# MaxWolf-01/sentinel2-landcover-classification

Hardware: AMD Instinct MI355X
Metric: Sentinel-2 256x256x13 tiles/sec fwd+bwd (higher is better)
Workload: dtype f32

## Files before the change

### sentinel2-landcover-classification_amd/csrc/ew.hip

```cpp
#include "common.h"

namespace s2k {

constexpr int CHUNK = 4096;

template <typename T>
static T* ref_ptr(const Ctx& c, int64_t ref) {
    if (ref < 0) return nullptr;
    const int base = (int)(ref >> 56);
    const int64_t off = ref & ((1ll << 56) - 1);
    if (base >= c.n_bases || c.bases[base] == nullptr) return reinterpret_cast<T*>(1);
    return reinterpret_cast<T*>(static_cast<char*>(c.bases[base]) + off);
}
static bool bad(const void* q) { return q == reinterpret_cast<const void*>(1); }
#define CHECK_PTRS(name, ...)                                                                         \
    do {                                                                                              \
        const void* _ps[] = {__VA_ARGS__};                                                            \
        for (const void* _q : _ps)                                                                    \
            if (bad(_q)) { set_error(name ": tensor references a null base"); return S2K_EFAULT; }    \
    } while (0)

struct Task {
    int64_t plane;
    int start, count;
// ... 998 lines not shown
    if (!dgate || !gate || !hpre || !pool || !w1 || !w2 || !dpool || !hs || B <= 0 || (params && (!dw1 || !db1 || !dw2 || !db2))) {
        set_error("se_fc_bwd: bad args"); return S2K_EINVAL;
    }
    if (Q > 8192 || B > 65535) { set_error("se_fc_bwd: C/Q too large"); return S2K_EINVAL; }
    if ((size_t)(C + 1024) * 4 > 64000) { set_error("se_fc_bwd: C too large"); return S2K_EINVAL; }
    if (Q <= 64) {
        hipLaunchKernelGGL(se_fc_bwd_small_kernel, dim3(B), dim3(1024), (size_t)(C + 1024 + 64) * sizeof(float), c.stream, dgate, gate, hpre, w1, w2,
                           hs, dpool, C, Q);
    } else {
    hipLaunchKernelGGL(se_fc_bwd_a1_kernel, dim3(cdiv(Q, 64), B), dim3(1024), (C + 1024) * sizeof(float), c.stream, dgate, gate, hpre, w2, hs, B, C, Q);
    hipLaunchKernelGGL(se_fc_bwd_a2_kernel, dim3(cdiv(C, NTHREADS), B), dim3(NTHREADS), Q * sizeof(float), c.stream, dgate, gate, hpre, w1, dpool, B, C, Q);
    }
    if (!params) return S2K_OK;
    launch_se_fc_param_grads(dgate, hs, hpre, pool, dw1, db1, dw2, db2, B, C, Q, c.stream);
    return S2K_OK;
}

int launch_se_fc_wgrad(const S2kOp& op, const Ctx& c) {
    const float* dgp = ref_ptr<const float>(c, op.t[S2K_SE_FC_WGRAD_T_DGP]);
    const float* hs = ref_ptr<const float>(c, op.t[S2K_SE_FC_WGRAD_T_HS]);
    const float* dhp = ref_ptr<const float>(c, op.t[S2K_SE_FC_WGRAD_T_DHP]);
    const float* pool = ref_ptr<const float>(c, op.t[S2K_SE_FC_WGRAD_T_POOL]);
    float* dw1 = ref_ptr<float>(c, op.t[S2K_SE_FC_WGRAD_T_DW1]);
    float* db1 = ref_ptr<float>(c, op.t[S2K_SE_FC_WGRAD_T_DB1]);
    float* dw2 = ref_ptr<float>(c, op.t[S2K_SE_FC_WGRAD_T_DW2]);
    float* db2 = ref_ptr<float>(c, op.t[S2K_SE_FC_WGRAD_T_DB2]);
    CHECK_PTRS("se_fc_wgrad", dgp, hs, dhp, pool, dw1, db1, dw2, db2);
    const int B = op.d[S2K_SE_FC_WGRAD_D_B], C = op.d[S2K_SE_FC_WGRAD_D_C], Q = op.d[S2K_SE_FC_WGRAD_D_CSQ];
    if (!dgp || !hs || !dhp || !pool || !dw1 || !db1 || !dw2 || !db2 || B <= 0 || C <= 0 || Q <= 0) { set_error("se_fc_wgrad: bad args"); return S2K_EINVAL; }
    launch_se_fc_param_grads(dgp, hs, dhp, pool, dw1, db1, dw2, db2, B, C, Q, c.stream);
    return S2K_OK;
}

template <bool VEC>
__global__ void __launch_bounds__(NTHREADS) bn_bwd_reduce_kernel(const float* g, const float* y, const float* bnv,
                                                                 const float* mulbc, const float* addbc, const float* noise,
                                                                 float* gout, double* stats2, int C, int HW, int64_t nplanes,
                                                                 int act, float keep, float addscale, int nrep) {
    Task t;
    if (!get_task(HW, nplanes, t)) return;
    const int lane = threadIdx.x & 63;
    const int c = (int)((uint32_t)t.plane % (uint32_t)C);
    const int b = (int)((uint32_t)t.plane / (uint32_t)C);
    const float scale = bnv[c], shift = bnv[C + c], mean = bnv[2 * C + c], invstd = bnv[3 * C + c];
    float mul = mulbc ? mulbc[t.plane] : 1.0f;
    if (noise) mul *= floorf(keep + noise[b]) / keep;
    const float add = addbc ? addbc[t.plane] * addscale : 0.0f;
    const int64_t base = t.plane * HW + t.start;
    float s1 = 0.0f, s2 = 0.0f;
    if (VEC) {
        const int n4 = t.count >> 2;
        for (int i = lane; i < n4; i += 64) {
            float4 gv = reinterpret_cast<const float4*>(g + base)[i];
            const float4 yv = reinterpret_cast<const float4*>(y + base)[i];
            float* gp = &gv.x;
            const float* yp = &yv.x;
#pragma unroll
            for (int k = 0; k < 4; ++k) {
                float v = fmaf(gp[k], mul, add);
                if (act != S2K_PRO_NONE) v *= act_grad(fmaf(yp[k], scale, shift), act);
                gp[k] = v;
                s1 += v;
                s2 = fmaf(v, (yp[k] - mean) * invstd, s2);
            }
            reinterpret_cast<float4*>(gout + base)[i] = gv;
        }
    } else {
        for (int i = lane; i < t.count; i += 64) {
            const float yy = y[base + i];
            float v = fmaf(g[base + i], mul, add);
            if (act != S2K_PRO_NONE) v *= act_grad(fmaf(yy, scale, shift), act);
            gout[base + i] = v;
            s1 += v;
            s2 = fmaf(v, (yy - mean) * invstd, s2);
        }
    }
    s1 = wave_sum(s1);
    s2 = wave_sum(s2);
    if (lane == 0) {
        double* st = stats2 + (int64_t)(blockIdx.x % nrep) * 2 * C;
        atomic_add_d(st + c, (double)s1);
        atomic_add_d(st + C + c, (double)s2);
    }
}

int launch_bn_bwd_reduce(const S2kOp& op, const Ctx& c) {
    const float* g = ref_ptr<const float>(c, op.t[S2K_BN_BWD_REDUCE_T_G]);
    const float* y = ref_ptr<const float>(c, op.t[S2K_BN_BWD_REDUCE_T_Y]);
    const float* bnv = ref_ptr<const float>(c, op.t[S2K_BN_BWD_REDUCE_T_BNV]);
    const float* mulbc = ref_ptr<const float>(c, op.t[S2K_BN_BWD_REDUCE_T_MULBC]);
    const float* addbc = ref_ptr<const float>(c, op.t[S2K_BN_BWD_REDUCE_T_ADDBC]);
    const float* noise = ref_ptr<const float>(c, op.t[S2K_BN_BWD_REDUCE_T_NOISE]);
    float* gout = ref_ptr<float>(c, op.t[S2K_BN_BWD_REDUCE_T_GOUT]);
    double* st2 = ref_ptr<double>(c, op.t[S2K_BN_BWD_REDUCE_T_STATS2]);
    CHECK_PTRS("bn_bwd_reduce", g, y, bnv, mulbc, addbc, noise, gout, st2);
    const int B = op.d[S2K_BN_BWD_REDUCE_D_B], C = op.d[S2K_BN_BWD_REDUCE_D_C], HW = op.d[S2K_BN_BWD_REDUCE_D_HW];
    if (!g || !y || !bnv || !gout || !st2 || B <= 0 || C <= 0 || HW <= 0) { set_error("bn_bwd_reduce: bad args"); return S2K_EINVAL; }
    const int64_t nplanes = (int64_t)B * C;
    const unsigned blocks = task_blocks(HW, nplanes);
    const int act = op.d[S2K_BN_BWD_REDUCE_D_ACT];
    const float keep = op.f[S2K_BN_BWD_REDUCE_F_KEEP], addscale = op.f[S2K_BN_BWD_REDUCE_F_ADDSCALE];
    const int nrep = op.d[S2K_BN_BWD_REDUCE_D_NREP] > 0 ? op.d[S2K_BN_BWD_REDUCE_D_NREP] : 1;
    if ((HW & 3) == 0)
        hipLaunchKernelGGL((bn_bwd_reduce_kernel<true>), dim3(blocks), dim3(NTHREADS), 0, c.stream, g, y, bnv, mulbc, addbc, noise,
                           gout, st2, C, HW, nplanes, act, keep, addscale, nrep);
    else
        hipLaunchKernelGGL((bn_bwd_reduce_kernel<false>), dim3(blocks), dim3(NTHREADS), 0, c.stream, g, y, bnv, mulbc, addbc, noise,
                           gout, st2, C, HW, nplanes, act, keep, addscale, nrep);
    return S2K_OK;
}

__global__ void bn_bwd_finalize_kernel(const double* st2, const float* gamma, const float* bnv, float* dgamma, float* dbeta,
                                       float* coef, int C, double count, int nrep) {
    const int c = blockIdx.x * 4 + (threadIdx.x >> 6);
    const int lane = threadIdx.x & 63;
    if (c >= C) return;
    double s1 = 0.0, s2 = 0.0;
    for (int r = lane; r < nrep; r += 64) { s1 += st2[(int64_t)r * 2 * C + c]; s2 += st2[(int64_t)r * 2 * C + C + c]; }
    s1 = wave_sum_d(s1);
    s2 = wave_sum_d(s2);
    if (lane != 0) return;
    dgamma[c] += (float)s2;
    dbeta[c] += (float)s1;
    const double a = (double)gamma[c] * (double)bnv[3 * C + c];
    coef[c] = (float)a;
    coef[C + c] = (float)(-a * s2 / count);
    coef[2 * C + c] = (float)(-a * s1 / count);
}

int launch_bn_bwd_finalize(const S2kOp& op, const Ctx& c) {
    const double* st2 = ref_ptr<const double>(c, op.t[S2K_BN_BWD_FINALIZE_T_STATS2]);
    const float* gamma = ref_ptr<const float>(c, op.t[S2K_BN_BWD_FINALIZE_T_GAMMA]);
    const float* bnv = ref_ptr<const float>(c, op.t[S2K_BN_BWD_FINALIZE_T_BNV]);
    float* dgamma = ref_ptr<float>(c, op.t[S2K_BN_BWD_FINALIZE_T_DGAMMA]);
    float* dbeta = ref_ptr<float>(c, op.t[S2K_BN_BWD_FINALIZE_T_DBETA]);
    float* coef = ref_ptr<float>(c, op.t[S2K_BN_BWD_FINALIZE_T_COEF]);
    CHECK_PTRS("bn_bwd_finalize", st2, gamma, bnv, dgamma, dbeta, coef);
    const int C = op.d[S2K_BN_BWD_FINALIZE_D_C];
    if (!st2 || !gamma || !bnv || !dgamma || !dbeta || !coef || C <= 0) { set_error("bn_bwd_finalize: bad args"); return S2K_EINVAL; }
    hipLaunchKernelGGL(bn_bwd_finalize_kernel, dim3(cdiv(C, 4)), dim3(256), 0, c.stream, st2, gamma, bnv, dgamma, dbeta, coef, C,
                       (double)op.n[S2K_BN_BWD_FINALIZE_N_COUNT], op.d[S2K_BN_BWD_FINALIZE_D_NREP] > 0 ? op.d[S2K_BN_BWD_FINALIZE_D_NREP] : 1);
    return S2K_OK;
}

struct BnFuse {
    const double* st2;
    const float* gamma;
    float *dgamma, *dbeta;
    double inv_count;
    int nrep;
    const float *mulbc, *addbc;
    float addscale;
    const float* ps;
    int B;
};

__device__ __forceinline__ void bn_fuse_sums(const BnFuse& fz, int C, int c, int lane, double& s1, double& s2) {
    s1 = 0.0; s2 = 0.0;
    if (fz.ps) {
        const int64_t np = (int64_t)fz.B * C;
        for (int b = lane; b < fz.B; b += 64) {
            const int64_t pl = (int64_t)b * C + c;
            const double mul = fz.mulbc ? (double)fz.mulbc[pl] : 1.0, add = fz.addbc ? (double)fz.addbc[pl] * (double)fz.addscale : 0.0;
            s1 += mul * (double)fz.ps[pl] + add * (double)fz.ps[np + pl];
            s2 += mul * (double)fz.ps[2 * np + pl] + add * (double)fz.ps[3 * np + pl];
        }
        s1 = wave_sum_d(s1);
        s2 = wave_sum_d(s2);
    } else if (fz.nrep <= 8) {
        for (int r = 0; r < fz.nrep; ++r) { s1 += fz.st2[(int64_t)r * 2 * C + c]; s2 += fz.st2[(int64_t)r * 2 * C + C + c]; }
    } else {
        for (int r = lane; r < fz.nrep; r += 64) { s1 += fz.st2[(int64_t)r * 2 * C + c]; s2 += fz.st2[(int64_t)r * 2 * C + C + c]; }
        s1 = wave_sum_d(s1);
        s2 = wave_sum_d(s2);
    }
}

__device__ __forceinline__ uint32_t pm_pk_bf16(float lo, float hi) {
    typedef __bf16 b2 __attribute__((ext_vector_type(2)));
    typedef float f2 __attribute__((ext_vector_type(2)));
    f2 v = {lo, hi};
    return __builtin_bit_cast(uint32_t, __builtin_convertvector(v, b2));
}

template <int MODE, bool VEC, bool OUT16 = false>
__global__ void __launch_bounds__(NTHREADS) plane_map_kernel(const float* a, const float* y, const float* bnv, const float* coef,
                                                             const float* noise, float* out, int C, int HW, int64_t nplanes,
                                                             float keep, const BnFuse fz, const BnFold fold = BnFold{}) {
    Task t;
    if (!get_task(HW, nplanes, t)) return;
    const int lane = threadIdx.x & 63;
    const int c = (int)((uint32_t)t.plane % (uint32_t)C);
    const int64_t base = t.plane * HW + t.start;
    float4 av0 = make_float4(0, 0, 0, 0), yv0 = make_float4(0, 0, 0, 0);
    if (VEC && lane < (t.count >> 2)) {
        if (a) av0 = reinterpret_cast<const float4*>(a + base)[lane];
        yv0 = reinterpret_cast<const float4*>(y + base)[lane];
    }
    float k0, k1, k2;
    float gmul = 1.0f, gadd = 0.0f, bscale = 1.0f, bshift = 0.0f;
    if (MODE == 3) {
        gmul = fz.mulbc ? fz.mulbc[t.plane] : 1.0f;
        gadd = fz.addbc ? fz.addbc[t.plane] * fz.addscale : 0.0f;
        bscale = bnv[c];
        bshift = bnv[C + c];
    }
    if (MODE >= 2) {
        double s1, s2;
        bn_fuse_sums(fz, C, c, lane, s1, s2);
        const float mean = bnv[2 * C + c], invstd = bnv[3 * C + c];
        const double aa = (double)fz.gamma[c] * (double)invstd;
        const float A = (float)aa, Bq = (float)(-aa * s2 * fz.inv_count), Cq = (float)(-aa * s1 * fz.inv_count);
        k0 = A; k1 = Bq * invstd; k2 = Cq - Bq * invstd * mean;
        if (t.plane < C && t.start == 0 && lane == 0) {
            fz.dgamma[c] += (float)s2;
            fz.dbeta[c] += (float)s1;
        }
    } else if (MODE == 0) {
        const float mean = bnv[2 * C + c], invstd = bnv[3 * C + c];
        const float A = coef[c], Bq = coef[C + c], Cq = coef[2 * C + c];
        k0 = A; k1 = Bq * invstd; k2 = Cq - Bq * invstd * mean;
    } else {
        float dcs = 1.0f;
        if (noise) dcs = floorf(keep + noise[(int)(t.plane / C)]) / keep;
        float sc, sh;
        if (fold.stats) bn_fold_wave(fold, C, c, t.plane < C && t.start == 0, sc, sh);
        else { sc = bnv[c]; sh = bnv[C + c]; }
        k0 = a ? 1.0f : 0.0f; k1 = sc * dcs; k2 = sh * dcs;
    }
    if (VEC) {
        const int n4 = t.count >> 2;
        for (int i = lane; i < n4; i += 64) {
            float4 av = av0, yv = yv0;
            if (i + 64 < n4) {
                if (a) av0 = reinterpret_cast<const float4*>(a + base)[i + 64];
                yv0 = reinterpret_cast<const float4*>(y + base)[i + 64];
            }
            if (MODE == 3) {
                av.x = fmaf(av.x, gmul, gadd) * act_grad(fmaf(yv.x, bscale, bshift), S2K_PRO_SILU);
                av.y = fmaf(av.y, gmul, gadd) * act_grad(fmaf(yv.y, bscale, bshift), S2K_PRO_SILU);
                av.z = fmaf(av.z, gmul, gadd) * act_grad(fmaf(yv.z, bscale, bshift), S2K_PRO_SILU);
                av.w = fmaf(av.w, gmul, gadd) * act_grad(fmaf(yv.w, bscale, bshift), S2K_PRO_SILU);
            }
            float4 o;
            o.x = fmaf(k0, av.x, fmaf(k1, yv.x, k2)); o.y = fmaf(k0, av.y, fmaf(k1, yv.y, k2));
            o.z = fmaf(k0, av.z, fmaf(k1, yv.z, k2)); o.w = fmaf(k0, av.w, fmaf(k1, yv.w, k2));
            if constexpr (OUT16) reinterpret_cast<uint2*>(reinterpret_cast<uint16_t*>(out) + base)[i] = make_uint2(pm_pk_bf16(o.x, o.y), pm_pk_bf16(o.z, o.w));
            else reinterpret_cast<float4*>(out + base)[i] = o;
        }
    } else {
        for (int i = lane; i < t.count; i += 64) {
            float av = a ? a[base + i] : 0.0f;
            if (MODE == 3) av = fmaf(av, gmul, gadd) * act_grad(fmaf(y[base + i], bscale, bshift), S2K_PRO_SILU);
            out[base + i] = fmaf(k0, av, fmaf(k1, y[base + i], k2));
        }
    }
}

template <int MODE, bool OUT16 = false>
__global__ void __launch_bounds__(NTHREADS) bn_bwd_apply_small_kernel(const float* a, const float* y, const float* bnv, float* out,
                                                                      int B, int C, int HW, int lpp, const BnFuse fz) {
    const int lane = threadIdx.x & 63;
    const int c = blockIdx.x * 4 + (threadIdx.x >> 6);
    if (c >= C) return;
    double s1, s2;
    bn_fuse_sums(fz, C, c, lane, s1, s2);
    const float mean = bnv[2 * C + c], invstd = bnv[3 * C + c];
    const double aa = (double)fz.gamma[c] * (double)invstd;
    const float A = (float)aa, Bq = (float)(-aa * s2 * fz.inv_count), Cq = (float)(-aa * s1 * fz.inv_count);
    const float k0 = A, k1 = Bq * invstd, k2 = Cq - Bq * invstd * mean;
    if (blockIdx.y == 0 && lane == 0) {
        fz.dgamma[c] += (float)s2;
        fz.dbeta[c] += (float)s1;
    }
    const float bscale = bnv[c], bshift = bnv[C + c];
    const int pp = 64 / lpp, sub = lane / lpp, li = lane & (lpp - 1);
    if (4 * li >= HW) return;
    const int bper = (B + gridDim.y - 1) / gridDim.y, b_lo = blockIdx.y * bper, b_hi = min(B, b_lo + bper);
    constexpr int U = 4;
    for (int b0 = b_lo + sub; b0 < b_hi; b0 += pp * U) {
        float4 av[U], yv[U];
        float gmul[U], gadd[U];
#pragma unroll
        for (int u = 0; u < U; ++u) {
            const int b = min(b0 + u * pp, b_hi - 1);
            const int64_t plane = (int64_t)b * C + c, off = plane * HW + 4 * li;
            av[u] = *reinterpret_cast<const float4*>(a + off);
            yv[u] = *reinterpret_cast<const float4*>(y + off);
            gmul[u] = 1.0f;
            gadd[u] = 0.0f;
            if (MODE == 3) {
                if (fz.mulbc) gmul[u] = fz.mulbc[plane];
                if (fz.addbc) gadd[u] = fz.addbc[plane] * fz.addscale;
            }
        }
#pragma unroll
        for (int u = 0; u < U; ++u) {
            const int b = b0 + u * pp;
            if (b >= b_hi) break;
            float4 g = av[u];
            const float4 yy = yv[u];
            if (MODE == 3) {
                g.x = fmaf(g.x, gmul[u], gadd[u]) * act_grad(fmaf(yy.x, bscale, bshift), S2K_PRO_SILU);
                g.y = fmaf(g.y, gmul[u], gadd[u]) * act_grad(fmaf(yy.y, bscale, bshift), S2K_PRO_SILU);
                g.z = fmaf(g.z, gmul[u], gadd[u]) * act_grad(fmaf(yy.z, bscale, bshift), S2K_PRO_SILU);
                g.w = fmaf(g.w, gmul[u], gadd[u]) * act_grad(fmaf(yy.w, bscale, bshift), S2K_PRO_SILU);
            }
            float4 o;
            o.x = fmaf(k0, g.x, fmaf(k1, yy.x, k2)); o.y = fmaf(k0, g.y, fmaf(k1, yy.y, k2));
            o.z = fmaf(k0, g.z, fmaf(k1, yy.z, k2)); o.w = fmaf(k0, g.w, fmaf(k1, yy.w, k2));
            if constexpr (OUT16) *reinterpret_cast<uint2*>(reinterpret_cast<uint16_t*>(out) + ((int64_t)b * C + c) * HW + 4 * li) = make_uint2(pm_pk_bf16(o.x, o.y), pm_pk_bf16(o.z, o.w));
            else *reinterpret_cast<float4*>(out + ((int64_t)b * C + c) * HW + 4 * li) = o;
        }
    }
}

template <int MODE, bool OUT16 = false>
static bool launch_bn_bwd_apply_small(const float* a, const float* y, const float* bnv, float* out, int B, int C, int HW,
                                      hipStream_t st, const BnFuse& fz) {
    if (HW > 64 || (HW & 3) || B < 2) return false;
    int lpp = 1;
    while (4 * lpp < HW) lpp <<= 1;
    const int bsplit = std::max(1, std::min(cdiv(B, 64 / lpp), cdiv(2048, C)));
    hipLaunchKernelGGL((bn_bwd_apply_small_kernel<MODE, OUT16>), dim3(cdiv(C, 4), bsplit), dim3(NTHREADS), 0, st, a, y, bnv, out, B, C, HW, lpp, fz);
    return true;
}

__global__ void __launch_bounds__(NTHREADS) bn_residual_small_kernel(const float* ident, const float* y, const float* bnv, const float* noise,
                                                                     float* out, int B, int C, int HW, float keep, int lpp,
                                                                     const BnFold fold) {
    const int lane = threadIdx.x & 63;
    const int c = blockIdx.x * 4 + (threadIdx.x >> 6);
    if (c >= C) return;
    float sc, sh;
    if (fold.stats) bn_fold_wave(fold, C, c, blockIdx.y == 0, sc, sh);
    else { sc = bnv[c]; sh = bnv[C + c]; }
    const int pp = 64 / lpp, sub = lane / lpp, li = lane & (lpp - 1);
    if (4 * li >= HW) return;
    const int bper = (B + gridDim.y - 1) / gridDim.y, b_lo = blockIdx.y * bper;
// ... 46 lines not shown
        launch_plane_map<0>(gp, y, bnv, coef, nullptr, dy, B, C, HW, 1.0f, c.stream);
        return S2K_OK;
    }
    fz.ps = ref_ptr<const float>(c, op.t[S2K_BN_BWD_APPLY_T_PS]);
    fz.B = B;
    if ((!fz.st2 && !fz.ps) || !fz.gamma || !fz.dgamma || !fz.dbeta || count <= 0) { set_error("bn_bwd_apply: fused form needs STATS2 (or PS), GAMMA, DGAMMA, DBETA, COUNT"); return S2K_EINVAL; }
    fz.mulbc = ref_ptr<const float>(c, op.t[S2K_BN_BWD_APPLY_T_MULBC]);
    fz.addbc = ref_ptr<const float>(c, op.t[S2K_BN_BWD_APPLY_T_ADDBC]);
    fz.addscale = op.f[S2K_BN_BWD_APPLY_F_ADDSCALE];
    CHECK_PTRS("bn_bwd_apply", fz.mulbc, fz.addbc, fz.ps);
    if (fz.ps && op.d[S2K_BN_BWD_APPLY_D_ACT] != S2K_PRO_SILU) { set_error("bn_bwd_apply: PS belongs to the recomputing (SiLU) form"); return S2K_EINVAL; }
    const bool out16 = op.d[S2K_BN_BWD_APPLY_D_OUT_BF16] != 0;
    if (out16 && (op.d[S2K_BN_BWD_APPLY_D_ACT] != S2K_PRO_NONE || fz.mulbc || fz.addbc || (HW & 3) || dy == gp)) {
        set_error("bn_bwd_apply: OUT_BF16 is for the plain fused form, HW % 4 == 0, out of place"); return S2K_EINVAL;
    }
    if (out16) {
        if (launch_bn_bwd_apply_small<2, true>(gp, y, bnv, dy, B, C, HW, c.stream, fz)) return S2K_OK;
        const int64_t nplanes = (int64_t)B * C;
        hipLaunchKernelGGL((plane_map_kernel<2, true, true>), dim3(task_blocks(HW, nplanes)), dim3(NTHREADS), 0, c.stream, gp, y, bnv,
                           (const float*)nullptr, (const float*)nullptr, dy, C, HW, nplanes, 1.0f, fz, BnFold{});
        return S2K_OK;
    }
    if (op.d[S2K_BN_BWD_APPLY_D_ACT] == S2K_PRO_NONE && !fz.mulbc && !fz.addbc) {
        if (launch_bn_bwd_apply_small<2>(gp, y, bnv, dy, B, C, HW, c.stream, fz)) return S2K_OK;
        launch_plane_map<2>(gp, y, bnv, nullptr, nullptr, dy, B, C, HW, 1.0f, c.stream, fz);
        return S2K_OK;
    }
    if (op.d[S2K_BN_BWD_APPLY_D_ACT] != S2K_PRO_SILU) { set_error("bn_bwd_apply: the recomputing form is SiLU only"); return S2K_EINVAL; }
    if (launch_bn_bwd_apply_small<3>(gp, y, bnv, dy, B, C, HW, c.stream, fz)) return S2K_OK;
    launch_plane_map<3>(gp, y, bnv, nullptr, nullptr, dy, B, C, HW, 1.0f, c.stream, fz);
    return S2K_OK;
}

int launch_bn_residual(const S2kOp& op, const Ctx& c) {
    const float* y = ref_ptr<const float>(c, op.t[S2K_BN_RESIDUAL_T_Y]);
    const float* bnv = ref_ptr<const float>(c, op.t[S2K_BN_RESIDUAL_T_BNV]);
    const float* ident = ref_ptr<const float>(c, op.t[S2K_BN_RESIDUAL_T_IDENT]);
    const float* noise = ref_ptr<const float>(c, op.t[S2K_BN_RESIDUAL_T_NOISE]);
    float* xout = ref_ptr<float>(c, op.t[S2K_BN_RESIDUAL_T_XOUT]);
    CHECK_PTRS("bn_residual", y, bnv, ident, noise, xout);
    if (!y || !bnv || !xout) { set_error("bn_residual: bad args"); return S2K_EINVAL; }
    BnFold fold;
    if (int e = fill_bn_fold(fold, c, &op.t[S2K_BN_RESIDUAL_T_FSTATS], op.n[S2K_BN_RESIDUAL_N_FCOUNT], op.d[S2K_BN_RESIDUAL_D_FNREP],
                             op.f[S2K_BN_RESIDUAL_F_FEPS], op.f[S2K_BN_RESIDUAL_F_FMOM], const_cast<float*>(bnv), "bn_residual")) return e;
    {
        const int B = op.d[S2K_BN_RESIDUAL_D_B], C = op.d[S2K_BN_RESIDUAL_D_C], HW = op.d[S2K_BN_RESIDUAL_D_HW];
        if (HW <= 256 && (HW & 3) == 0 && B > 1) {
            int lpp = 1;
            while (4 * lpp < HW) lpp <<= 1;
            const int bsplit = std::max(1, std::min(cdiv(B, 64 / lpp), cdiv(2048, C)));
            hipLaunchKernelGGL(bn_residual_small_kernel, dim3(cdiv(C, 4), bsplit), dim3(NTHREADS), 0, c.stream, ident, y, bnv, noise, xout, B, C, HW,
                               op.f[S2K_BN_RESIDUAL_F_KEEP], lpp, fold);
            return S2K_OK;
        }
    }
    launch_plane_map<1>(ident, y, bnv, nullptr, noise, xout, op.d[S2K_BN_RESIDUAL_D_B], op.d[S2K_BN_RESIDUAL_D_C],
                        op.d[S2K_BN_RESIDUAL_D_HW], op.f[S2K_BN_RESIDUAL_F_KEEP], c.stream, BnFuse{}, fold);
    return S2K_OK;
}

__global__ void __launch_bounds__(NTHREADS) space_to_depth_kernel(const float* x, float* y, int C, int H, int W, int64_t total) {
    const int64_t i = (int64_t)blockIdx.x * NTHREADS + threadIdx.x;
    if (i >= total) return;
    const int wq = W >> 2;
    const int xq = (int)(i % wq);
    int64_t r = i / wq;
// ... 163 lines not shown
```

### sentinel2-landcover-classification_amd/csrc/s2k_api.hip

```cpp
#include <cstdarg>
#include <cstdio>
#include <cstring>
#include <mutex>
#include <vector>

#include <stdlib.h>

#include "common.h"

namespace s2k {

static thread_local char g_err[512] = "";
thread_local int g_s2k_variant = 0;

void set_error(const char* fmt, ...) {
    va_list ap;
    va_start(ap, fmt);
    vsnprintf(g_err, sizeof(g_err), fmt, ap);
    va_end(ap);
}

int launch_conv(const S2kOp&, const Ctx&);
int launch_wgrad(const S2kOp&, const Ctx&);
int launch_dwconv_fwd(const S2kOp&, const Ctx&);
int launch_dwconv_dgrad(const S2kOp&, const Ctx&);
int launch_dwconv_wgrad(const S2kOp&, const Ctx&);
int launch_axpy(const S2kOp&, const Ctx&);
int launch_weight_pack(const S2kOp&, const Ctx&);
int launch_wgrad_finalize(const S2kOp&, const Ctx&);
int launch_bn_finalize(const S2kOp&, const Ctx&);
int launch_se_pool(const S2kOp&, const Ctx&);
int launch_se_fc(const S2kOp&, const Ctx&);
int launch_se_fc_bwd(const S2kOp&, const Ctx&);
int launch_se_bwd_reduce(const S2kOp&, const Ctx&);
int launch_bn_bwd_reduce(const S2kOp&, const Ctx&);
int launch_bn_bwd_finalize(const S2kOp&, const Ctx&);
int launch_bn_bwd_apply(const S2kOp&, const Ctx&);
int launch_bn_residual(const S2kOp&, const Ctx&);
int launch_channel_sum(const S2kOp&, const Ctx&);
int launch_loss_fwd(const S2kOp&, const Ctx&);
int launch_loss_bwd(const S2kOp&, const Ctx&);
int launch_argmax(const S2kOp&, const Ctx&);
int launch_chan_ln_fwd(const S2kOp&, const Ctx&);
int launch_chan_ln_bwd(const S2kOp&, const Ctx&);
int launch_act_bwd(const S2kOp&, const Ctx&);
int launch_act_fwd(const S2kOp&, const Ctx&);
int launch_attn_fwd(const S2kOp&, const Ctx&);
int launch_attn_bwd(const S2kOp&, const Ctx&);
int launch_mae_mask_index(const S2kOp&, const Ctx&);
int launch_token_gather(const S2kOp&, const Ctx&);
int launch_token_scatter(const S2kOp&, const Ctx&);
int launch_patchify(const S2kOp&, const Ctx&);
int launch_mae_loss_fwd(const S2kOp&, const Ctx&);
int launch_mae_loss_bwd(const S2kOp&, const Ctx&);
int launch_transpose_cl(const S2kOp&, const Ctx&);
int launch_drop_gate(const S2kOp&, const Ctx&);
int launch_confusion(const S2kOp&, const Ctx&);
int launch_tile_prep(const S2kOp&, const Ctx&);
int launch_se_bn_sums(const S2kOp&, const Ctx&);
int launch_se_bn_combine(const S2kOp&, const Ctx&);
int launch_space_to_depth(const S2kOp&, const Ctx&);
int launch_se_fc_wgrad(const S2kOp&, const Ctx&);
int launch_ids_to_dec_idx(const S2kOp&, const Ctx&);
int launch_upsample_zero(const S2kOp&, const Ctx&);
int launch_im2col(const S2kOp&, const Ctx&);
int launch_adam(float*, const float*, float*, float*, int64_t, double, double, double, double, double, int, hipStream_t);
int launch_mfma_selftest(const float*, const float*, float*, hipStream_t);

static int launch_memset(const S2kOp& op, const Ctx& c) {
    const int64_t ref = op.t[S2K_MEMSET_T_DST];
// ... 42 lines not shown
        case S2K_OP_BN_BWD_APPLY: return launch_bn_bwd_apply(op, c);
        case S2K_OP_BN_RESIDUAL: return launch_bn_residual(op, c);
        case S2K_OP_CHANNEL_SUM: return launch_channel_sum(op, c);
        case S2K_OP_LOSS_FWD: return launch_loss_fwd(op, c);
        case S2K_OP_LOSS_BWD: return launch_loss_bwd(op, c);
        case S2K_OP_ARGMAX: return launch_argmax(op, c);
        case S2K_OP_CHAN_LN_FWD: return launch_chan_ln_fwd(op, c);
        case S2K_OP_CHAN_LN_BWD: return launch_chan_ln_bwd(op, c);
        case S2K_OP_ACT_BWD: return launch_act_bwd(op, c);
        case S2K_OP_ACT_FWD: return launch_act_fwd(op, c);
        case S2K_OP_ATTN_FWD: return launch_attn_fwd(op, c);
        case S2K_OP_ATTN_BWD: return launch_attn_bwd(op, c);
        case S2K_OP_MAE_MASK_INDEX: return launch_mae_mask_index(op, c);
        case S2K_OP_TOKEN_GATHER: return launch_token_gather(op, c);
        case S2K_OP_TOKEN_SCATTER: return launch_token_scatter(op, c);
        case S2K_OP_PATCHIFY: return launch_patchify(op, c);
        case S2K_OP_MAE_LOSS_FWD: return launch_mae_loss_fwd(op, c);
        case S2K_OP_MAE_LOSS_BWD: return launch_mae_loss_bwd(op, c);
        case S2K_OP_TRANSPOSE_CL: return launch_transpose_cl(op, c);
        case S2K_OP_DROP_GATE: return launch_drop_gate(op, c);
        case S2K_OP_CONFUSION: return launch_confusion(op, c);
        case S2K_OP_TILE_PREP: return launch_tile_prep(op, c);
        case S2K_OP_SE_BN_SUMS: return launch_se_bn_sums(op, c);
        case S2K_OP_SE_BN_COMBINE: return launch_se_bn_combine(op, c);
        case S2K_OP_SPACE_TO_DEPTH: return launch_space_to_depth(op, c);
        case S2K_OP_SE_FC_WGRAD: return launch_se_fc_wgrad(op, c);
        case S2K_OP_IDS_TO_DEC_IDX: return launch_ids_to_dec_idx(op, c);
        case S2K_OP_UPSAMPLE_ZERO: return launch_upsample_zero(op, c);
        case S2K_OP_IM2COL: return launch_im2col(op, c);
        default: set_error("unknown stage kind %d", op.kind); return S2K_ENOSYS;
    }
}

static int check_launch(int rc, const S2kOp& op, int index) {
    if (rc != S2K_OK) {
        char tmp[400];
        snprintf(tmp, sizeof(tmp), "%s", g_err);
        set_error("op %d (%s): %s", index, (op.kind > 0 && op.kind <= S2K_N_KINDS) ? kNames[op.kind] : "?", tmp);
        return rc;
    }
    const hipError_t e = hipGetLastError();
    if (e != hipSuccess) {
        set_error("op %d (%s): HIP launch error: %s", index, (op.kind > 0 && op.kind <= S2K_N_KINDS) ? kNames[op.kind] : "?",
                  hipGetErrorString(e));
        return S2K_EHIP;
    }
    return S2K_OK;
}

}

using namespace s2k;

extern "C" {

int s2k_abi_version(void) { return S2K_ABI_VERSION; }
size_t s2k_op_size(void) { return sizeof(S2kOp); }
const char* s2k_last_error(void) { return g_err; }
const char* s2k_kind_name(int kind) { return (kind > 0 && kind <= S2K_N_KINDS) ? kNames[kind] : nullptr; }

struct SideQueue {
    hipStream_t stream = nullptr;
    hipEvent_t fork = nullptr, join = nullptr;
};
constexpr int kMaxDevices = 64;
static std::mutex g_pool_mu;
// ... 36 lines not shown
struct DeviceGuard {
    int prev = -1, dev = -1;
    bool switched = false;
    explicit DeviceGuard(hipStream_t st) {
        if (hipGetDevice(&prev) != hipSuccess) prev = -1;
        dev = prev;
        int sd = -1;
        if (st != nullptr && hipStreamGetDevice(st, &sd) == hipSuccess && sd >= 0) dev = sd;
        (void)hipGetLastError();
        if (dev != prev && dev >= 0) switched = hipSetDevice(dev) == hipSuccess;
    }
    ~DeviceGuard() {
        if (switched && prev >= 0) (void)hipSetDevice(prev);
    }
};

int s2k_program_run(const S2kOp* ops, int begin, int end, void* const* bases, int n_bases, void* stream) {
    if (!ops || !bases || begin < 0 || end < begin) { set_error("program_run: bad arguments"); return S2K_EINVAL; }
    hipStream_t main_st = static_cast<hipStream_t>(stream);
    DeviceGuard guard(main_st);
    Ctx c{bases, n_bases, main_st};
    bool any_side = false;
    for (int i = begin; i < end && !any_side; ++i) any_side = (ops[i].flags & S2K_FLAG_SIDE) != 0;
    SideQueue* sq = any_side ? lease_side_queue(guard.dev) : nullptr;
    bool side_busy = false;
    bool main_dirty = true;
    auto join = [&]() {
        if (!side_busy) return;
        (void)hipEventRecord(sq->join, sq->stream);
        (void)hipStreamWaitEvent(main_st, sq->join, 0);
        side_busy = false;
    };
    int rc = S2K_OK;
    for (int i = begin; i < end; ++i) {
        const S2kOp& op = ops[i];
        if ((op.flags & S2K_FLAG_SIDE) && sq) {
            if (main_dirty) {
                (void)hipEventRecord(sq->fork, main_st);
                (void)hipStreamWaitEvent(sq->stream, sq->fork, 0);
                main_dirty = false;
            }
            Ctx cs{bases, n_bases, sq->stream};
            rc = check_launch(dispatch(op, cs), op, i);
            side_busy = true;
        } else {
            if (op.flags & S2K_FLAG_JOIN) join();
            rc = check_launch(dispatch(op, c), op, i);
            main_dirty = true;
        }
        if (rc != S2K_OK) break;
    }
    join();
    release_side_queue(guard.dev, sq);
    return rc;
}

int s2k_op_launch(const S2kOp* op, void* const* bases, int n_bases, void* stream) {
    if (!op || !bases) { set_error("op_launch: bad arguments"); return S2K_EINVAL; }
    DeviceGuard guard(static_cast<hipStream_t>(stream));
    Ctx c{bases, n_bases, static_cast<hipStream_t>(stream)};
    return check_launch(dispatch(*op, c), *op, 0);
}

static int profile_impl(const S2kOp* ops, int begin, int end, void* const* bases, int n_bases, void* stream, float* ms_by_kind,
                        int* launches_by_kind, float* ms_per_op, int* variant_per_op);

int s2k_program_profile(const S2kOp* ops, int begin, int end, void* const* bases, int n_bases, void* stream, float* ms_by_kind,
                        int* launches_by_kind) {
    return profile_impl(ops, begin, end, bases, n_bases, stream, ms_by_kind, launches_by_kind, nullptr, nullptr);
}

int s2k_program_profile_ops(const S2kOp* ops, int begin, int end, void* const* bases, int n_bases, void* stream,
                            float* ms_per_op) {
    float ms[S2K_N_KINDS + 1];
    int cnt[S2K_N_KINDS + 1];
    return profile_impl(ops, begin, end, bases, n_bases, stream, ms, cnt, ms_per_op, nullptr);
}

int s2k_program_profile_variants(const S2kOp* ops, int begin, int end, void* const* bases, int n_bases, void* stream,
                                 float* ms_per_op, int* variant_per_op) {
    float ms[S2K_N_KINDS + 1];
    int cnt[S2K_N_KINDS + 1];
    if (!ms_per_op || !variant_per_op) { set_error("program_profile_variants: bad arguments"); return S2K_EINVAL; }
    return profile_impl(ops, begin, end, bases, n_bases, stream, ms, cnt, ms_per_op, variant_per_op);
}

static int profile_impl(const S2kOp* ops, int begin, int end, void* const* bases, int n_bases, void* stream, float* ms_by_kind,
                        int* launches_by_kind, float* ms_per_op, int* variant_per_op) {
    if (!ops || !bases || !ms_by_kind || !launches_by_kind || begin < 0 || end < begin) {
        set_error("program_profile: bad arguments");
        return S2K_EINVAL;
    }
    hipStream_t st = static_cast<hipStream_t>(stream);
    DeviceGuard guard(st);
    Ctx c{bases, n_bases, st};
    const int n = end - begin;
    hipEvent_t* ev = new hipEvent_t[n + 1];
    for (int i = 0; i <= n; ++i) hipEventCreate(&ev[i]);
    int rc = S2K_OK;
    hipEventRecord(ev[0], st);
    int done = 0;
    for (int i = 0; i < n; ++i) {
        g_s2k_variant = 0;
        rc = check_launch(dispatch(ops[begin + i], c), ops[begin + i], begin + i);
        if (rc != S2K_OK) break;
        if (variant_per_op) variant_per_op[i] = g_s2k_variant;
        hipEventRecord(ev[i + 1], st);
        done = i + 1;
    }
    hipStreamSynchronize(st);
    if (rc == S2K_OK) {
        for (int k = 0; k <= S2K_N_KINDS; ++k) { ms_by_kind[k] = 0.0f; launches_by_kind[k] = 0; }
        for (int i = 0; i < done; ++i) {
            float ms = 0.0f;
            hipEventElapsedTime(&ms, ev[i], ev[i + 1]);
            const int k = ops[begin + i].kind;
            if (ms_per_op) ms_per_op[i] = ms;
            if (k > 0 && k <= S2K_N_KINDS) { ms_by_kind[k] += ms; launches_by_kind[k] += 1; }
        }
    }
    for (int i = 0; i <= n; ++i) hipEventDestroy(ev[i]);
    delete[] ev;
    return rc;
}

int s2k_adam_step(float* p, const float* g, float* m, float* v, int64_t n, double lr, double beta1, double beta2, double eps,
                  double weight_decay, int step, void* stream) {
    DeviceGuard guard(static_cast<hipStream_t>(stream));
    const int rc = launch_adam(p, g, m, v, n, lr, beta1, beta2, eps, weight_decay, step, static_cast<hipStream_t>(stream));
    if (rc != S2K_OK) return rc;
    const hipError_t e = hipGetLastError();
    if (e != hipSuccess) { set_error("adam: %s", hipGetErrorString(e)); return S2K_EHIP; }
    return S2K_OK;
}

int s2k_selftest_mfma(const float* a, const float* b, float* d, void* stream) {
    if (!a || !b || !d) { set_error("selftest: null pointer"); return S2K_EINVAL; }
// ... 9 lines not shown
```

Baseline: 989.4.

## Fuse BN backward reduce/apply pairs, skipping the intermediate gradient write

Consecutive BN_BWD_REDUCE and BN_BWD_APPLY ops are detected at dispatch time and run as a pair. For small B*HW a single per-channel kernel holds g and y in registers, reduces, finalizes the stats and writes the output in one pass. Otherwise the reduce runs without storing gout and the apply recomputes the pre-BN gradient from g, including ReLU, mul/add broadcast and drop-path noise. This removes one full write and read of the gradient tensor, and for small layers one or two launches, at the cost of extra recompute, register pressure and more complex dispatch logic.

```diff
diff --git a/sentinel2-landcover-classification_amd/csrc/ew.hip b/sentinel2-landcover-classification_amd/csrc/ew.hip
--- a/sentinel2-landcover-classification_amd/csrc/ew.hip
+++ b/sentinel2-landcover-classification_amd/csrc/ew.hip
@@ -1054,7 +1054,7 @@
     return S2K_OK;
 }
 
-template <bool VEC>
+template <bool VEC, bool WRITE = true>
 __global__ void __launch_bounds__(NTHREADS) bn_bwd_reduce_kernel(const float* g, const float* y, const float* bnv,
                                                                  const float* mulbc, const float* addbc, const float* noise,
                                                                  float* gout, double* stats2, int C, int HW, int64_t nplanes,
@@ -1085,14 +1085,14 @@
                 s1 += v;
                 s2 = fmaf(v, (yp[k] - mean) * invstd, s2);
             }
-            reinterpret_cast<float4*>(gout + base)[i] = gv;
+            if (WRITE) reinterpret_cast<float4*>(gout + base)[i] = gv;
         }
     } else {
         for (int i = lane; i < t.count; i += 64) {
             const float yy = y[base + i];
             float v = fmaf(g[base + i], mul, add);
             if (act != S2K_PRO_NONE) v *= act_grad(fmaf(yy, scale, shift), act);
-            gout[base + i] = v;
+            if (WRITE) gout[base + i] = v;
             s1 += v;
             s2 = fmaf(v, (yy - mean) * invstd, s2);
         }
@@ -1106,7 +1106,7 @@
     }
 }
 
-int launch_bn_bwd_reduce(const S2kOp& op, const Ctx& c) {
+static int bn_bwd_reduce_impl(const S2kOp& op, const Ctx& c, bool write) {
     const float* g = ref_ptr<const float>(c, op.t[S2K_BN_BWD_REDUCE_T_G]);
     const float* y = ref_ptr<const float>(c, op.t[S2K_BN_BWD_REDUCE_T_Y]);
     const float* bnv = ref_ptr<const float>(c, op.t[S2K_BN_BWD_REDUCE_T_BNV]);
@@ -1123,14 +1123,21 @@
     const int act = op.d[S2K_BN_BWD_REDUCE_D_ACT];
     const float keep = op.f[S2K_BN_BWD_REDUCE_F_KEEP], addscale = op.f[S2K_BN_BWD_REDUCE_F_ADDSCALE];
     const int nrep = op.d[S2K_BN_BWD_REDUCE_D_NREP] > 0 ? op.d[S2K_BN_BWD_REDUCE_D_NREP] : 1;
-    if ((HW & 3) == 0)
-        hipLaunchKernelGGL((bn_bwd_reduce_kernel<true>), dim3(blocks), dim3(NTHREADS), 0, c.stream, g, y, bnv, mulbc, addbc, noise,
-                           gout, st2, C, HW, nplanes, act, keep, addscale, nrep);
-    else
-        hipLaunchKernelGGL((bn_bwd_reduce_kernel<false>), dim3(blocks), dim3(NTHREADS), 0, c.stream, g, y, bnv, mulbc, addbc, noise,
-                           gout, st2, C, HW, nplanes, act, keep, addscale, nrep);
-    return S2K_OK;
-}
+#define S2K_BN_REDUCE_LAUNCH(VEC, WRITE)                                                                                          \
+    hipLaunchKernelGGL((bn_bwd_reduce_kernel<VEC, WRITE>), dim3(blocks), dim3(NTHREADS), 0, c.stream, g, y, bnv, mulbc, addbc, \
+                       noise, gout, st2, C, HW, nplanes, act, keep, addscale, nrep)
+    if ((HW & 3) == 0) {
+        if (write) S2K_BN_REDUCE_LAUNCH(true, true);
+        else S2K_BN_REDUCE_LAUNCH(true, false);
+    } else {
+        if (write) S2K_BN_REDUCE_LAUNCH(false, true);
+        else S2K_BN_REDUCE_LAUNCH(false, false);
+    }
+#undef S2K_BN_REDUCE_LAUNCH
+    return S2K_OK;
+}
+
+int launch_bn_bwd_reduce(const S2kOp& op, const Ctx& c) { return bn_bwd_reduce_impl(op, c, true); }
 
 __global__ void bn_bwd_finalize_kernel(const double* st2, const float* gamma, const float* bnv, float* dgamma, float* dbeta,
                                        float* coef, int C, double count, int nrep) {
@@ -1175,7 +1182,21 @@
     float addscale;
     const float* ps;
     int B;
+    const float* noise;
+    float keep;
+    int act;
 };
+
+__device__ __forceinline__ void bn_pair_plane(const BnFuse& fz, int64_t plane, int b, float& mul, float& add) {
+    mul = fz.mulbc ? fz.mulbc[plane] : 1.0f;
+    if (fz.noise) mul *= floorf(fz.keep + fz.noise[b]) / fz.keep;
+    add = fz.addbc ? fz.addbc[plane] * fz.addscale : 0.0f;
+}
+__device__ __forceinline__ float bn_pair_gp(float g, float y, float mul, float add, float scale, float shift, bool relu) {
+    float v = fmaf(g, mul, add);
+    if (relu) v *= fmaf(y, scale, shift) > 0.0f ? 1.0f : 0.0f;
+    return v;
+}
 
 __device__ __forceinline__ void bn_fuse_sums(const BnFuse& fz, int C, int c, int lane, double& s1, double& s2) {
     s1 = 0.0; s2 = 0.0;
@@ -1227,6 +1248,12 @@
         bscale = bnv[c];
         bshift = bnv[C + c];
     }
+    if (MODE == 4) {
+        bn_pair_plane(fz, t.plane, (int)((uint32_t)t.plane / (uint32_t)C), gmul, gadd);
+        bscale = bnv[c];
+        bshift = bnv[C + c];
+    }
+    const bool relu = MODE == 4 && fz.act == S2K_PRO_RELU;
     if (MODE >= 2) {
         double s1, s2;
         bn_fuse_sums(fz, C, c, lane, s1, s2);
@@ -1264,6 +1291,12 @@
                 av.z = fmaf(av.z, gmul, gadd) * act_grad(fmaf(yv.z, bscale, bshift), S2K_PRO_SILU);
                 av.w = fmaf(av.w, gmul, gadd) * act_grad(fmaf(yv.w, bscale, bshift), S2K_PRO_SILU);
             }
+            if (MODE == 4) {
+                av.x = bn_pair_gp(av.x, yv.x, gmul, gadd, bscale, bshift, relu);
+                av.y = bn_pair_gp(av.y, yv.y, gmul, gadd, bscale, bshift, relu);
+                av.z = bn_pair_gp(av.z, yv.z, gmul, gadd, bscale, bshift, relu);
+                av.w = bn_pair_gp(av.w, yv.w, gmul, gadd, bscale, bshift, relu);
+            }
             float4 o;
             o.x = fmaf(k0, av.x, fmaf(k1, yv.x, k2)); o.y = fmaf(k0, av.y, fmaf(k1, yv.y, k2));
             o.z = fmaf(k0, av.z, fmaf(k1, yv.z, k2)); o.w = fmaf(k0, av.w, fmaf(k1, yv.w, k2));
@@ -1274,6 +1307,7 @@
         for (int i = lane; i < t.count; i += 64) {
             float av = a ? a[base + i] : 0.0f;
             if (MODE == 3) av = fmaf(av, gmul, gadd) * act_grad(fmaf(y[base + i], bscale, bshift), S2K_PRO_SILU);
+            if (MODE == 4) av = bn_pair_gp(av, y[base + i], gmul, gadd, bscale, bshift, relu);
             out[base + i] = fmaf(k0, av, fmaf(k1, y[base + i], k2));
         }
     }
@@ -1315,6 +1349,7 @@
                 if (fz.mulbc) gmul[u] = fz.mulbc[plane];
                 if (fz.addbc) gadd[u] = fz.addbc[plane] * fz.addscale;
             }
+            if (MODE == 4) bn_pair_plane(fz, plane, b, gmul[u], gadd[u]);
         }
 #pragma unroll
         for (int u = 0; u < U; ++u) {
@@ -1327,6 +1362,13 @@
                 g.y = fmaf(g.y, gmul[u], gadd[u]) * act_grad(fmaf(yy.y, bscale, bshift), S2K_PRO_SILU);
                 g.z = fmaf(g.z, gmul[u], gadd[u]) * act_grad(fmaf(yy.z, bscale, bshift), S2K_PRO_SILU);
                 g.w = fmaf(g.w, gmul[u], gadd[u]) * act_grad(fmaf(yy.w, bscale, bshift), S2K_PRO_SILU);
+            }
+            if (MODE == 4) {
+                const bool relu = fz.act == S2K_PRO_RELU;
+                g.x = bn_pair_gp(g.x, yy.x, gmul[u], gadd[u], bscale, bshift, relu);
+                g.y = bn_pair_gp(g.y, yy.y, gmul[u], gadd[u], bscale, bshift, relu);
+                g.z = bn_pair_gp(g.z, yy.z, gmul[u], gadd[u], bscale, bshift, relu);
+                g.w = bn_pair_gp(g.w, yy.w, gmul[u], gadd[u], bscale, bshift, relu);
             }
             float4 o;
             o.x = fmaf(k0, g.x, fmaf(k1, yy.x, k2)); o.y = fmaf(k0, g.y, fmaf(k1, yy.y, k2));
@@ -1439,6 +1481,137 @@
     return S2K_OK;
 }
 
+constexpr int BN_PAIR_LAZY = 1, BN_PAIR_RESIDENT = 2;
+constexpr int BN_RESIDENT_MAX = 2048;
+
+int bn_bwd_pair_route(int B, int C, int HW, int act) {
+    if (B <= 0 || C <= 0 || HW <= 0 || (act != S2K_PRO_NONE && act != S2K_PRO_RELU)) return 0;
+    static const int resident_max = tune_int("S2K_BN_RESIDENT_MAX", BN_RESIDENT_MAX);
+    if ((HW & 3) == 0 && B >= 2 && (int64_t)B * HW <= std::min(resident_max, BN_RESIDENT_MAX)) return BN_PAIR_RESIDENT;
+    return BN_PAIR_LAZY;
+}
+
+__global__ void __launch_bounds__(NTHREADS) bn_bwd_channel_kernel(const float* g, const float* y, const float* bnv, float* out,
+                                                                  double* st2w, int B, int C, int HW, const BnFuse fz) {
+    const int lane = threadIdx.x & 63;
+    const int c = __builtin_amdgcn_readfirstlane(blockIdx.x * 4 + (threadIdx.x >> 6));
+    if (c >= C) return;
+    constexpr int U = BN_RESIDENT_MAX / 256;
+    const uint32_t hw4 = (uint32_t)HW >> 2, n4 = (uint32_t)B * hw4;
+    float4 gv[U], yv[U];
+    float gmul[U], gadd[U];
+    int64_t off[U];
+#pragma unroll
+    for (int u = 0; u < U; ++u) {
+        if ((uint32_t)(64 * u) < n4) {
+            const uint32_t j = min((uint32_t)(lane + 64 * u), n4 - 1);
+            const uint32_t b = j / hw4, q = j - b * hw4;
+            const int64_t plane = (int64_t)b * C + c;
+            off[u] = plane * HW + 4 * q;
+            gv[u] = *reinterpret_cast<const float4*>(g + off[u]);
+            yv[u] = *reinterpret_cast<const float4*>(y + off[u]);
+            bn_pair_plane(fz, plane, (int)b, gmul[u], gadd[u]);
+        }
+    }
+    double p1, p2;
+    bn_fuse_sums(fz, C, c, lane, p1, p2);
+    const float scale = bnv[c], shift = bnv[C + c], mean = bnv[2 * C + c], invstd = bnv[3 * C + c];
+    const bool relu = fz.act == S2K_PRO_RELU;
+    float s1 = 0.0f, s2 = 0.0f;
+#pragma unroll
+    for (int u = 0; u < U; ++u) {
+        if ((uint32_t)(64 * u) < n4 && (uint32_t)(lane + 64 * u) < n4) {
+            float* gp = &gv[u].x;
+            const float* yp = &yv[u].x;
+#pragma unroll
+            for (int k = 0; k < 4; ++k) {
+                const float v = bn_pair_gp(gp[k], yp[k], gmul[u], gadd[u], scale, shift, relu);
+                gp[k] = v;
+                s1 += v;
+                s2 = fmaf(v, (yp[k] - mean) * invstd, s2);
+            }
+        }
+    }
+    const double d1 = wave_sum_d((double)s1), d2 = wave_sum_d((double)s2);
+    const double t1 = p1 + d1, t2 = p2 + d2;
+    if (lane == 0) {
+        st2w[c] += d1;
+        st2w[C + c] += d2;
+        fz.dgamma[c] += (float)t2;
+        fz.dbeta[c] += (float)t1;
+    }
+    const double aa = (double)fz.gamma[c] * (double)invstd;
+    const float A = (float)aa, Bq = (float)(-aa * t2 * fz.inv_count), Cq = (float)(-aa * t1 * fz.inv_count);
+    const float k0 = A, k1 = Bq * invstd, k2 = Cq - Bq * invstd * mean;
+#pragma unroll
+    for (int u = 0; u < U; ++u) {
+        if ((uint32_t)(64 * u) < n4 && (uint32_t)(lane + 64 * u) < n4) {
+            const float4 gg = gv[u], yy = yv[u];
+            float4 o;
+            o.x = fmaf(k0, gg.x, fmaf(k1, yy.x, k2)); o.y = fmaf(k0, gg.y, fmaf(k1, yy.y, k2));
+            o.z = fmaf(k0, gg.z, fmaf(k1, yy.z, k2)); o.w = fmaf(k0, gg.w, fmaf(k1, yy.w, k2));
+            *reinterpret_cast<float4*>(out + off[u]) = o;
+        }
+    }
+}
+
+static int bn_pair_fuse(const S2kOp& red, const S2kOp& app, const Ctx& c, BnFuse& fz) {
+    fz = BnFuse{};
+    fz.st2 = ref_ptr<const double>(c, app.t[S2K_BN_BWD_APPLY_T_STATS2]);
+    fz.gamma = ref_ptr<const float>(c, app.t[S2K_BN_BWD_APPLY_T_GAMMA]);
+    fz.dgamma = ref_ptr<float>(c, app.t[S2K_BN_BWD_APPLY_T_DGAMMA]);
+    fz.dbeta = ref_ptr<float>(c, app.t[S2K_BN_BWD_APPLY_T_DBETA]);
+    const double count = (double)app.n[S2K_BN_BWD_APPLY_N_COUNT];
+    fz.inv_count = (count > 0 && !app.d[S2K_BN_BWD_APPLY_D_EVAL]) ? 1.0 / count : 0.0;
+    fz.nrep = app.d[S2K_BN_BWD_APPLY_D_NREP] > 0 ? app.d[S2K_BN_BWD_APPLY_D_NREP] : 1;
+    fz.B = app.d[S2K_BN_BWD_APPLY_D_B];
+    fz.mulbc = ref_ptr<const float>(c, red.t[S2K_BN_BWD_REDUCE_T_MULBC]);
+    fz.addbc = ref_ptr<const float>(c, red.t[S2K_BN_BWD_REDUCE_T_ADDBC]);
+    fz.addscale = red.f[S2K_BN_BWD_REDUCE_F_ADDSCALE];
+    fz.noise = ref_ptr<const float>(c, red.t[S2K_BN_BWD_REDUCE_T_NOISE]);
+    fz.keep = red.f[S2K_BN_BWD_REDUCE_F_KEEP];
+    fz.act = red.d[S2K_BN_BWD_REDUCE_D_ACT];
+    CHECK_PTRS("bn_bwd_pair", fz.st2, fz.gamma, fz.dgamma, fz.dbeta, fz.mulbc, fz.addbc, fz.noise);
+    if (!fz.st2 || !fz.gamma || !fz.dgamma || !fz.dbeta || count <= 0) { set_error("bn_bwd_pair: the fused APPLY needs STATS2, GAMMA, DGAMMA, DBETA, COUNT"); return S2K_EINVAL; }
+    return S2K_OK;
+}
+
+int launch_bn_bwd_pair_head(const S2kOp& red, const S2kOp& app, const Ctx& c, int form) {
+    g_s2k_variant = form;
+    if (form == BN_PAIR_LAZY) return bn_bwd_reduce_impl(red, c, false);
+    const float* g = ref_ptr<const float>(c, red.t[S2K_BN_BWD_REDUCE_T_G]);
+    const float* y = ref_ptr<const float>(c, red.t[S2K_BN_BWD_REDUCE_T_Y]);
+    const float* bnv = ref_ptr<const float>(c, red.t[S2K_BN_BWD_REDUCE_T_BNV]);
+    double* st2 = ref_ptr<double>(c, red.t[S2K_BN_BWD_REDUCE_T_STATS2]);
+    float* dy = ref_ptr<float>(c, app.t[S2K_BN_BWD_APPLY_T_DY]);
+    CHECK_PTRS("bn_bwd_pair", g, y, bnv, st2, dy);
+    const int B = red.d[S2K_BN_BWD_REDUCE_D_B], C = red.d[S2K_BN_BWD_REDUCE_D_C], HW = red.d[S2K_BN_BWD_REDUCE_D_HW];
+    if (!g || !y || !bnv || !st2 || !dy || form != BN_PAIR_RESIDENT || (HW & 3) || (int64_t)B * HW > BN_RESIDENT_MAX) {
+        set_error("bn_bwd_pair: bad args"); return S2K_EINVAL;
+    }
+    BnFuse fz;
+    if (int e = bn_pair_fuse(red, app, c, fz)) return e;
+    hipLaunchKernelGGL(bn_bwd_channel_kernel, dim3(cdiv(C, 4)), dim3(NTHREADS), 0, c.stream, g, y, bnv, dy, st2, B, C, HW, fz);
+    return S2K_OK;
+}
+
+int launch_bn_bwd_pair_apply(const S2kOp& red, const S2kOp& app, const Ctx& c, int form) {
+    g_s2k_variant = form;
+    if (form == BN_PAIR_RESIDENT) return S2K_OK;
+    const float* g = ref_ptr<const float>(c, red.t[S2K_BN_BWD_REDUCE_T_G]);
+    const float* y = ref_ptr<const float>(c, app.t[S2K_BN_BWD_APPLY_T_Y]);
+    const float* bnv = ref_ptr<const float>(c, app.t[S2K_BN_BWD_APPLY_T_BNV]);
+    float* dy = ref_ptr<float>(c, app.t[S2K_BN_BWD_APPLY_T_DY]);
+    CHECK_PTRS("bn_bwd_pair", g, y, bnv, dy);
+    if (!g || !y || !bnv || !dy || form != BN_PAIR_LAZY) { set_error("bn_bwd_pair: bad args"); return S2K_EINVAL; }
+    BnFuse fz;
+    if (int e = bn_pair_fuse(red, app, c, fz)) return e;
+    const int B = app.d[S2K_BN_BWD_APPLY_D_B], C = app.d[S2K_BN_BWD_APPLY_D_C], HW = app.d[S2K_BN_BWD_APPLY_D_HW];
+    if (launch_bn_bwd_apply_small<4>(g, y, bnv, dy, B, C, HW, c.stream, fz)) return S2K_OK;
+    launch_plane_map<4>(g, y, bnv, nullptr, nullptr, dy, B, C, HW, 1.0f, c.stream, fz);
+    return S2K_OK;
+}
+
 int launch_bn_residual(const S2kOp& op, const Ctx& c) {
     const float* y = ref_ptr<const float>(c, op.t[S2K_BN_RESIDUAL_T_Y]);
     const float* bnv = ref_ptr<const float>(c, op.t[S2K_BN_RESIDUAL_T_BNV]);
diff --git a/sentinel2-landcover-classification_amd/csrc/s2k_api.hip b/sentinel2-landcover-classification_amd/csrc/s2k_api.hip
--- a/sentinel2-landcover-classification_amd/csrc/s2k_api.hip
+++ b/sentinel2-landcover-classification_amd/csrc/s2k_api.hip
@@ -36,6 +36,9 @@
 int launch_bn_bwd_reduce(const S2kOp&, const Ctx&);
 int launch_bn_bwd_finalize(const S2kOp&, const Ctx&);
 int launch_bn_bwd_apply(const S2kOp&, const Ctx&);
+int bn_bwd_pair_route(int B, int C, int HW, int act);
+int launch_bn_bwd_pair_head(const S2kOp& reduce, const S2kOp& apply, const Ctx&, int form);
+int launch_bn_bwd_pair_apply(const S2kOp& reduce, const S2kOp& apply, const Ctx&, int form);
 int launch_bn_residual(const S2kOp&, const Ctx&);
 int launch_channel_sum(const S2kOp&, const Ctx&);
 int launch_loss_fwd(const S2kOp&, const Ctx&);
@@ -144,6 +147,41 @@
     }
 }
 
+static bool bn_pairs_enabled() {
+    static const bool on = [] {
+        const char* e = getenv("S2K_NO_BN_PAIR");
+        return !(e && atoi(e) != 0);
+    }();
+    return on;
+}
+
+static int bn_pair_form(const S2kOp* ops, int i, int end) {
+    if (i + 1 >= end || !bn_pairs_enabled()) return 0;
+    const S2kOp& r = ops[i];
+    const S2kOp& a = ops[i + 1];
+    if (r.kind != S2K_OP_BN_BWD_REDUCE || a.kind != S2K_OP_BN_BWD_APPLY) return 0;
+    if (a.t[S2K_BN_BWD_APPLY_T_COEF] >= 0 || a.t[S2K_BN_BWD_APPLY_T_PS] >= 0) return 0;
+    if ((r.flags & S2K_FLAG_SIDE) || (a.flags & (S2K_FLAG_SIDE | S2K_FLAG_JOIN))) return 0;
+    const int64_t gp = a.t[S2K_BN_BWD_APPLY_T_GP];
+    if (gp < 0 || gp != r.t[S2K_BN_BWD_REDUCE_T_GOUT] || a.t[S2K_BN_BWD_APPLY_T_DY] != gp) return 0;
+    if (a.d[S2K_BN_BWD_APPLY_D_OUT_BF16]) return 0;
+    if (a.t[S2K_BN_BWD_APPLY_T_Y] != r.t[S2K_BN_BWD_REDUCE_T_Y] || a.t[S2K_BN_BWD_APPLY_T_BNV] != r.t[S2K_BN_BWD_REDUCE_T_BNV] ||
+        a.t[S2K_BN_BWD_APPLY_T_STATS2] != r.t[S2K_BN_BWD_REDUCE_T_STATS2] || a.t[S2K_BN_BWD_APPLY_T_STATS2] < 0) return 0;
+    if (a.d[S2K_BN_BWD_APPLY_D_B] != r.d[S2K_BN_BWD_REDUCE_D_B] || a.d[S2K_BN_BWD_APPLY_D_C] != r.d[S2K_BN_BWD_REDUCE_D_C] ||
+        a.d[S2K_BN_BWD_APPLY_D_HW] != r.d[S2K_BN_BWD_REDUCE_D_HW] || a.d[S2K_BN_BWD_APPLY_D_NREP] != r.d[S2K_BN_BWD_REDUCE_D_NREP]) return 0;
+    if (a.d[S2K_BN_BWD_APPLY_D_ACT] != S2K_PRO_NONE || a.t[S2K_BN_BWD_APPLY_T_MULBC] >= 0 || a.t[S2K_BN_BWD_APPLY_T_ADDBC] >= 0) return 0;
+    return bn_bwd_pair_route(r.d[S2K_BN_BWD_REDUCE_D_B], r.d[S2K_BN_BWD_REDUCE_D_C], r.d[S2K_BN_BWD_REDUCE_D_HW], r.d[S2K_BN_BWD_REDUCE_D_ACT]);
+}
+
+static int run_stage(const S2kOp* ops, int i, int end, const Ctx& c, int& pair) {
+    const int form = pair;
+    pair = 0;
+    if (form) return launch_bn_bwd_pair_apply(ops[i - 1], ops[i], c, form);
+    if (ops[i].kind == S2K_OP_BN_BWD_REDUCE && (pair = bn_pair_form(ops, i, end)) != 0)
+        return launch_bn_bwd_pair_head(ops[i], ops[i + 1], c, pair);
+    return dispatch(ops[i], c);
+}
+
 static int check_launch(int rc, const S2kOp& op, int index) {
     if (rc != S2K_OK) {
         char tmp[400];
@@ -246,6 +284,7 @@
         side_busy = false;
     };
     int rc = S2K_OK;
+    int pair = 0;
     for (int i = begin; i < end; ++i) {
         const S2kOp& op = ops[i];
         if ((op.flags & S2K_FLAG_SIDE) && sq) {
@@ -255,11 +294,11 @@
                 main_dirty = false;
             }
             Ctx cs{bases, n_bases, sq->stream};
-            rc = check_launch(dispatch(op, cs), op, i);
+            rc = check_launch(run_stage(ops, i, end, cs, pair), op, i);
             side_busy = true;
         } else {
             if (op.flags & S2K_FLAG_JOIN) join();
-            rc = check_launch(dispatch(op, c), op, i);
+            rc = check_launch(run_stage(ops, i, end, c, pair), op, i);
             main_dirty = true;
         }
         if (rc != S2K_OK) break;
@@ -314,9 +353,10 @@
     int rc = S2K_OK;
     hipEventRecord(ev[0], st);
     int done = 0;
+    int pair = 0;
     for (int i = 0; i < n; ++i) {
         g_s2k_variant = 0;
-        rc = check_launch(dispatch(ops[begin + i], c), ops[begin + i], begin + i);
+        rc = check_launch(run_stage(ops, begin + i, end, c, pair), ops[begin + i], begin + i);
         if (rc != S2K_OK) break;
         if (variant_per_op) variant_per_op[i] = g_s2k_variant;
         hipEventRecord(ev[i + 1], st);
```

Result: no change. 997.3 (median of 6 runs) (+0.8%).
